# raulmur/ORB_SLAM2

Hardware: AMD Instinct MI355X
Metric: frames/s ORB extract+match, 1241x376 gray, 2000 kpts, 8 lvls (higher is better)
Workload: dtype u8

## Files before the change

orb_slam2_amd/csrc/orbhip_api.hip:

```cpp
#include <cstdarg>
#include <unistd.h>
#include <sys/syscall.h>
#include "orbhip_ctx.h"

static thread_local std::string g_err;
orbhip_status orbhip_set_error(orbhip_status st, const char* fmt, ...)
{
    char buf[512]; va_list ap; va_start(ap, fmt); vsnprintf(buf, sizeof buf, fmt, ap); va_end(ap);
    g_err = buf; return st;
}

static const char* kKernelNames[K_COUNT] = {"k_pyramid_level", "k_fast_cells", "k_blur", "k_quadtree", "k_describe",
                                            "k_match_grid", "k_match_candidates", "k_match_select", "k_undistort_keys", "k_remap"};

static const signed char kPatternHost[256 * 4] = {
#include "brief_pattern_31.inc"
};

void prof_collect(orbhip_ctx* c)
{
    for (auto& s : c->pending) {
        (void)hipEventSynchronize(s.b);
        float ms = 0; (void)hipEventElapsedTime(&ms, s.a, s.b);
        c->tot_ms[s.k] += ms; c->launches[s.k] += s.counts;
// ... 557 lines not shown

orbhip_status run_pipeline(orbhip_ctx* c, int nimg, const uint8_t* d_img0, long long frame_stride, int row_stride,
                           int match_prev, int window, float nnratio, int check_ori)
{
    orbhip_status st = begin_batch(c, d_img0, frame_stride, row_stride); if (st != ORBHIP_OK) return st;
    const int cur = c->cur, prev = (cur + 2) % 3;
    const int ngroups = std::min((int)c->xstreams.size() + 1, nimg);
    ExtractParams P = make_params(c, d_img0, frame_stride, row_stride);
    if (ngroups > 1) { HIPCHK(hipEventRecord(c->ev_fork, c->stream)); }
    for (int gi = 0; gi < ngroups; gi++) {
        const int f0 = (int)((long long)nimg * gi / ngroups), f1 = (int)((long long)nimg * (gi + 1) / ngroups), nf = f1 - f0;
        hipStream_t s = gi == 0 ? c->stream : c->xstreams[gi - 1];
        if (gi > 0) HIPCHK(hipStreamWaitEvent(s, c->ev_fork, 0));
        if (nf <= 0) continue;
        st = pipeline_frames(c, P, f0, nf, s, ngroups == 1); if (st != ORBHIP_OK) return st;
        if (gi > 0) { HIPCHK(hipEventRecord(c->xevents[gi - 1], s)); HIPCHK(hipStreamWaitEvent(c->stream, c->xevents[gi - 1], 0)); }
    }
    if (match_prev) {
        MatchParams M; memset(&M, 0, sizeof M);
        M.kp1 = c->distorted ? c->d_out_kpun[prev] : c->d_out_kp[prev]; M.desc1 = c->d_out_desc[prev]; M.n1 = c->d_out_n[prev]; M.n1_lvl0 = c->d_lvl_n[prev];
        M.kp2 = c->distorted ? c->d_out_kpun[cur] : c->d_out_kp[cur]; M.desc2 = c->d_out_desc[cur]; M.n2 = c->d_out_n[cur];
        M.lvl_stride = c->L; M.list1 = nullptr; M.prev_from_kp1 = 1;
        M.cap = c->out_cap; M.min_x = c->bounds.min_x; M.min_y = c->bounds.min_y; M.max_x = c->bounds.max_x; M.max_y = c->bounds.max_y;
        M.grid_start = c->d_grid_start; M.grid_items = c->d_grid_items; M.grid_xy = c->d_grid_xy; M.cand = c->d_cand; M.top = c->d_top; M.ncand = c->d_ncand; M.cand_stride = c->lvl0_cap; M.lvl0_cap = c->lvl0_cap;
        M.prev = c->d_prev; M.matches12 = c->d_m12; M.nmatches = c->d_nm; M.window = window; M.nnratio = nnratio; M.check_ori = check_ori; M.slot0 = 0;
        if (orbhip_match_select_big(c->out_cap, c->lvl0_cap)) {
            if (!c->d_match_ws) HIPCHK(dalloc(&c->d_match_ws, (size_t)c->B * orbhip_match_select_ints(c->out_cap, c->lvl0_cap)));
            M.big_ws = c->d_match_ws;
        }
        hipStream_t ms = c->serial ? c->stream : c->mstream;
        HIPCHK(hipEventRecord(c->ev_extract, c->stream));
        HIPCHK(hipStreamWaitEvent(ms, c->ev_extract, 0));
        { ProfScope ps(c, K_MGRID, ms); orbhip_launch_match_grid(M, nimg, ms); }
        { ProfScope ps(c, K_MCAND, ms); orbhip_launch_match_candidates(M, nimg, ms); }
        { ProfScope ps(c, K_MSELECT, ms); orbhip_launch_match_select(M, nimg, ms); }
        HIPCHK(hipEventRecord(c->ev_match[cur], ms));
        c->match_pending[cur] = true;
    }
    c->last_matched = match_prev != 0;
    c->last_nimg = nimg;
    HIPCHK(hipGetLastError());
    return ORBHIP_OK;
}

extern "C" orbhip_status orbhip_extract_device(orbhip_ctx* c, int nimg, const uint8_t* d_imgs, size_t frame_stride, int row_stride,
                                               int match_prev, int window, float nnratio, int check_ori)
{
    if (!c || !d_imgs) return fail(ORBHIP_ERR_INVALID, "null argument");
    if (nimg < 1 || nimg > c->B) return fail(ORBHIP_ERR_INVALID, "nimg %d outside 1..%d", nimg, c->B);
    if (row_stride < c->cfg.width) return fail(ORBHIP_ERR_INVALID, "row stride %d < width %d", row_stride, c->cfg.width);
// ... 133 lines not shown
```

orb_slam2_amd/csrc/orbhip_internal.h:

```cpp
#pragma once
#include <hip/hip_runtime.h>
#include <cstdint>
#include "../../include/orbhip.h"

#include <cstdlib>
inline hipError_t orbhip_dmalloc(void** p, size_t bytes)
{
    const hipError_t e = hipMalloc(p, bytes);
    if (e != hipSuccess) return e;
    static const int poison = [] { const char* v = getenv("ORBHIP_POISON"); return v && *v ? atoi(v) & 255 : -1; }();
    if (poison < 0) return hipSuccess;
    const hipError_t m = hipMemset(*p, poison, bytes);
    return m != hipSuccess ? m : hipDeviceSynchronize();
}

#define ORBHIP_MAX_LEVELS 16
#define ORBHIP_QT_DEPTH 13
#define ORBHIP_GRID_COLS 64
#define ORBHIP_GRID_ROWS 48
#define ORBHIP_GRID_CELLS (ORBHIP_GRID_COLS * ORBHIP_GRID_ROWS)
#define ORBHIP_HISTO_LENGTH 30
#define ORBHIP_TH_LOW 50
#define ORBHIP_EDGE 16

// ... 43 lines not shown
    const float* patternf;
    int iniTh, minTh, blur_round_mode, fp_contract;
    int qt_maxn;
    int qt_maxcells;
    int qt_scr;
    int fc_pstride, fc_prows, fc_sstride, fc_srows, fc_listcap;
    int fc_cell0, fc_ncells;
    int fc_pbytes, fc_np; const int4* fc_dma;
    const short2* pc_xr; const short2* pc_yr; int pc_ntx, pc_nty, pc_buf0, pc_buf1, pc_xcap, pc_ycap;
};

struct MatchParams {
    const orbhip_keypoint* kp1; const uint8_t* desc1; const int* n1;
    const int* n1_lvl0; int lvl_stride;
    const int* list1;
    int prev_from_kp1;
    const orbhip_keypoint* kp2; const uint8_t* desc2; const int* n2;
    int cap;
    float min_x, min_y, max_x, max_y;
    int* grid_start; int* grid_items; float2* grid_xy;
    unsigned* cand; int* ncand; int cand_stride;
    unsigned* top;
    int lvl0_cap;
    float* prev;
    int* matches12; int* nmatches;
    int window; float nnratio; int check_ori;
    int slot0;
    int grid_all_levels;
    int* big_ws;
};
size_t orbhip_match_select_ints(int cap, int lvl0_cap);
bool orbhip_match_select_big(int cap, int lvl0_cap);

struct StereoSide {
    const orbhip_keypoint* kp; const uint8_t* desc; const int* n;
    const uint8_t* img0; long long img0_frame_stride; int img0_pitch;
    const uint8_t* pyr; long long plane_frame_bytes;
};
struct StereoParams {
    const LevelGeom* geom; StereoSide L, R;
    int cap, im_h;
    int* row_start; int* row_items; int row_cap;
    float* u_right; float* depth; int* sad;
    float mbf, maxD;
};
hipError_t orbhip_copy_async(void* dst, const void* src, size_t bytes, hipMemcpyKind kind, hipStream_t s);
int orbhip_device_numa_node(int device);
bool orbhip_bind_thread_to_node(int node);
void orbhip_launch_stereo(const StereoParams& T, int nslots, int max_left, hipStream_t s, bool rows_ready = false);
void orbhip_launch_stereo_rows(const StereoParams& T, int nslots, hipStream_t s);

struct ProjParams {
    const orbhip_keypoint* kp; const uint8_t* desc; const float* u_right; int n;
    float min_x, min_y, max_x, max_y;
    const int* grid_start; const int* grid_items; const float2* grid_xy;
// ... 142 lines not shown
```

orb_slam2_amd/csrc/orbhip_kernels_match.hip:

```cpp
#include "orbhip_internal.h"
#include <cstdlib>
#include <cstring>
#include <type_traits>

#define WAVE 64
#define IMAX 0x7fffffff

#define NN_T 256
#define NN_QPT 4
#define NN_ROWS 256
#define NN_CHUNK 8192

struct NNPart { int best, second; long long idx; };

__global__ __launch_bounds__(NN_T) void k_hamming_nn(const unsigned long long* q, int nq, const unsigned long long* db, long long ndb,
                                                     long long base, NNPart* parts, int nchunks)
{
    __shared__ unsigned long long s_db[NN_ROWS * 4];
    const int tid = threadIdx.x, chunk = blockIdx.y;
    const int q0 = (blockIdx.x * NN_T + tid) * NN_QPT;
    unsigned long long qa[NN_QPT][4];
    unsigned kb[NN_QPT], ks[NN_QPT];
#pragma unroll
    for (int k = 0; k < NN_QPT; k++) {
// ... 444 lines not shown
    const float gwInv = (float)ORBHIP_GRID_COLS / (float)(M.max_x - M.min_x), ghInv = (float)ORBHIP_GRID_ROWS / (float)(M.max_y - M.min_y);
    size_t lds_max = (size_t)150 * 1024;
#ifdef ORBHIP_TEST_HOOKS
    if (const char* e = getenv("ORBHIP_TEST_MATCH_GRID_LDS_MAX")) lds_max = (size_t)atol(e);
#endif
    if (orbhip_match_grid_lds(M.cap) <= lds_max) hipLaunchKernelGGL(k_match_grid, dim3(nslots, 1, 1), dim3(256, 1, 1), orbhip_match_grid_lds(M.cap), s, M, gwInv, ghInv);
    else hipLaunchKernelGGL(k_match_grid_big, dim3(nslots, 1, 1), dim3(256, 1, 1), 0, s, M, gwInv, ghInv);
}

__device__ __forceinline__ int wave_min_dpp(int v)
{
    v = min(v, __builtin_amdgcn_update_dpp(IMAX, v, 0x111, 0xf, 0xf, false));
    v = min(v, __builtin_amdgcn_update_dpp(IMAX, v, 0x112, 0xf, 0xf, false));
    v = min(v, __builtin_amdgcn_update_dpp(IMAX, v, 0x114, 0xf, 0xe, false));
    v = min(v, __builtin_amdgcn_update_dpp(IMAX, v, 0x118, 0xf, 0xc, false));
    v = min(v, __builtin_amdgcn_update_dpp(IMAX, v, 0x142, 0xa, 0xf, false));
    v = min(v, __builtin_amdgcn_update_dpp(IMAX, v, 0x143, 0xc, 0xf, false));
    return __builtin_amdgcn_readlane(v, 63);
}

#define MS_K 4
#define MS_REC (MS_K + 1)
#define MS_NONE 0xFFFFFFFFu
#define MC_CHUNKS 8
__global__ __launch_bounds__(256) void k_match_candidates(MatchParams M, float gwInv, float ghInv)
{
    const int wave = __builtin_amdgcn_readfirstlane(threadIdx.x >> 6), lane = threadIdx.x & 63, slot = blockIdx.y + M.slot0;
    const int j1 = blockIdx.x * 4 + wave;
    const int n1l = M.n1_lvl0[slot * M.lvl_stride];
    if (j1 >= n1l || j1 >= M.lvl0_cap) return;
    const int i1 = M.list1 ? M.list1[(long long)slot * M.lvl0_cap + j1] : j1;
    const int nitems = M.grid_start[(long long)slot * (ORBHIP_GRID_CELLS + 1) + ORBHIP_GRID_CELLS];
    const int* gitems = M.grid_items + (long long)slot * M.cap;
    const float2* gxy = M.grid_xy + (long long)slot * M.cap;
    unsigned* cand = M.cand + ((long long)slot * M.lvl0_cap + j1) * M.cand_stride;
    const orbhip_keypoint* kp1 = M.kp1 + (long long)slot * M.cap;
    const float x = M.prev_from_kp1 ? kp1[i1].x : M.prev[((long long)slot * M.cap + i1) * 2];
    const float y = M.prev_from_kp1 ? kp1[i1].y : M.prev[((long long)slot * M.cap + i1) * 2 + 1];
    const float r = (float)M.window;
    const unsigned long long* d1 = (const unsigned long long*)(M.desc1 + ((long long)slot * M.cap + i1) * 32);
    const unsigned long long q0 = d1[0], q1 = d1[1], q2 = d1[2], q3 = d1[3];
    const unsigned long long below = (1ull << lane) - 1ull;
    int nc = 0;
    int tk[MS_K]; unsigned te[MS_K]; int nsel = 0;
#pragma unroll
    for (int k = 0; k < MS_K; k++) { tk[k] = IMAX; te[k] = MS_NONE; }
    const int* gstart = M.grid_start + (long long)slot * (ORBHIP_GRID_CELLS + 1);
    const float cl = __fmul_rn(__fsub_rn(__fsub_rn(x, M.min_x), r), gwInv), ch = __fmul_rn(__fadd_rn(__fsub_rn(x, M.min_x), r), gwInv);
    const int col_lo = cl >= 1.0f ? (int)fminf(floorf(cl) - 1.0f, (float)ORBHIP_GRID_COLS) : 0;
    const int col_hi = ch < (float)(ORBHIP_GRID_COLS - 2) ? (int)fmaxf(ceilf(ch) + 2.0f, 0.0f) : ORBHIP_GRID_COLS;
    const int t_lo = __builtin_amdgcn_readfirstlane(gstart[min(col_lo, col_hi) * ORBHIP_GRID_ROWS]), t_hi = __builtin_amdgcn_readfirstlane(gstart[col_hi * ORBHIP_GRID_ROWS]);
    (void)nitems;
    for (int tb = t_lo; tb < t_hi; tb += 64 * MC_CHUNKS) {
        float2 k[MC_CHUNKS]; int it[MC_CHUNKS];
#pragma unroll
        for (int c = 0; c < MC_CHUNKS; c++) {
            const int t = tb + 64 * c + lane;
            k[c].x = 0.0f; k[c].y = 0.0f; it[c] = 0;
            if (t < t_hi) { k[c] = gxy[t]; it[c] = gitems[t]; }
        }
#pragma unroll
        for (int c = 0; c < MC_CHUNKS; c++) {
            if (tb + 64 * c >= t_hi) break;
            const bool ok = tb + 64 * c + lane < t_hi && fabsf(__fsub_rn(k[c].x, x)) < r && fabsf(__fsub_rn(k[c].y, y)) < r;
            const unsigned long long m = __ballot(ok);
            if (m == 0) continue;
            const int pos = nc + __popcll(m & below);
            if (ok && pos < M.cand_stride) {
                const unsigned long long* d2 = (const unsigned long long*)(M.desc2 + ((long long)slot * M.cap + it[c]) * 32);
                const int dist = __popcll(q0 ^ d2[0]) + __popcll(q1 ^ d2[1]) + __popcll(q2 ^ d2[2]) + __popcll(q3 ^ d2[3]);
                unsigned rec = (unsigned)it[c] | ((unsigned)dist << 20);
                cand[pos] = rec;
                int key = (dist << 20) | pos;
                nsel++;
#pragma unroll
                for (int k = 0; k < MS_K; k++) if (key < tk[k]) { const int tkk = tk[k]; const unsigned tee = te[k]; tk[k] = key; te[k] = rec; key = tkk; rec = tee; }
            }
            nc += __popcll(m);
        }
    }
    nc = min(nc, M.cand_stride);
    if (lane == 0) M.ncand[(long long)slot * M.lvl0_cap + j1] = nc;
    unsigned out = MS_NONE; int popped = 0;
#pragma unroll
    for (int r = 0; r < MS_K; r++) {
        const int m = wave_min_dpp(tk[0]);
        if (m == IMAX) break;
        const int owner = __ffsll((long long)__ballot(tk[0] == m)) - 1;
        const unsigned rec = (unsigned)__builtin_amdgcn_readlane((int)te[0], owner);
        if (lane == r) out = rec;
        if (lane == owner) {
            popped++;
#pragma unroll
            for (int k = 0; k + 1 < MS_K; k++) { tk[k] = tk[k + 1]; te[k] = te[k + 1]; }
            tk[MS_K - 1] = IMAX; te[MS_K - 1] = MS_NONE;
        }
    }
    const bool more = __ballot(nsel > popped) != 0ull;
    unsigned* top = M.top + ((long long)slot * M.lvl0_cap + j1) * MS_REC;
    if (lane < MS_K) top[lane] = out;
    if (lane == MS_K) top[MS_K] = more ? 1u : 0u;
}

void orbhip_launch_match_candidates(const MatchParams& M, int nslots, hipStream_t s)
{
    const float gwInv = (float)ORBHIP_GRID_COLS / (float)(M.max_x - M.min_x), ghInv = (float)ORBHIP_GRID_ROWS / (float)(M.max_y - M.min_y);
    hipLaunchKernelGGL(k_match_candidates, dim3((M.lvl0_cap + 3) / 4, nslots, 1), dim3(256, 1, 1), 0, s, M, gwInv, ghInv);
}


#define MS_T 256

__device__ __forceinline__ int orbhip_match_select_ints_d(int cap, int lvl0_cap) { return 4 * cap + 4 * lvl0_cap + ORBHIP_HISTO_LENGTH + 8; }
template <bool BIG> __device__ __forceinline__ void match_select_body(const MatchParams& M)
{
    typedef typename std::conditional<BIG, volatile int, int>::type TI;
    typedef typename std::conditional<BIG, volatile float, float>::type TF;
    const int slot = blockIdx.x + M.slot0, tid = threadIdx.x, lane = tid & 63, wave = tid >> 6;
    const int n1 = M.n1[slot], n2 = M.n2[slot];
    const int n1l = min(M.n1_lvl0[slot * M.lvl_stride], M.lvl0_cap);
    const int* list1 = M.list1 ? M.list1 + (long long)slot * M.lvl0_cap : nullptr;
    HIP_DYNAMIC_SHARED(int, lds)
    TI* s_md = BIG ? M.big_ws + (long long)(blockIdx.x + M.slot0) * (long long)orbhip_match_select_ints_d(M.cap, M.lvl0_cap) : lds;
    TI* s_m21 = s_md + M.cap;
    TI* s_m12 = s_m21 + M.cap;
    TI* s_bin = s_m12 + M.lvl0_cap;
    TI* s_nc = s_bin + M.lvl0_cap;
    TI* s_hist = s_nc + M.lvl0_cap;
    TI* s_stamp = s_hist + ORBHIP_HISTO_LENGTH + 8;
    TF* s_ang1 = reinterpret_cast<TF*>(s_stamp + M.cap);
    TF* s_ang2 = s_ang1 + M.lvl0_cap;
    auto amin = [](TI* p, int v) { atomicMin(const_cast<int*>(p), v); };
    auto aadd = [](TI* p, int v) { atomicAdd(const_cast<int*>(p), v); };
    const orbhip_keypoint* kp1 = M.kp1 + (long long)slot * M.cap;
    const orbhip_keypoint* kp2 = M.kp2 + (long long)slot * M.cap;
    int* m12 = M.matches12 + (long long)slot * M.cap;
    float* prev = M.prev + (long long)slot * M.cap * 2;
    const unsigned* cand0 = M.cand + (long long)slot * M.lvl0_cap * M.cand_stride;
    for (int i = tid; i < n2; i += MS_T) { s_md[i] = IMAX; s_m21[i] = -1; s_stamp[i] = IMAX; s_ang2[i] = kp2[i].angle; }
    for (int i = tid; i < n1l; i += MS_T) { s_m12[i] = -1; s_bin[i] = -1; s_nc[i] = M.ncand[(long long)slot * M.lvl0_cap + i]; s_ang1[i] = kp1[list1 ? list1[i] : i].angle; }
    for (int i = tid; i < ORBHIP_HISTO_LENGTH + 8; i += MS_T) s_hist[i] = 0;
    for (int i = tid; i < n1; i += MS_T) { m12[i] = -1; if (M.prev_from_kp1) { prev[2 * i] = kp1[i].x; prev[2 * i + 1] = kp1[i].y; } }
    __syncthreads();
    if (wave == 0) {
        const float factor = 1.0f / ORBHIP_HISTO_LENGTH;
        const unsigned* top0 = M.top + (long long)slot * M.lvl0_cap * MS_REC;
        auto rot_bin = [&](int j1, int i2) -> int {
            float rot = __fsub_rn(s_ang1[j1], s_ang2[i2]);
            if (rot < 0.0f) rot = __fadd_rn(rot, 360.0f);
            int bin = (int)roundf(__fmul_rn(rot, factor));
            if (bin == ORBHIP_HISTO_LENGTH) bin = 0;
            return min(max(bin, 0), ORBHIP_HISTO_LENGTH - 1);
        };
        for (int jb = 0; jb < n1l; jb += 64) {
            const int j1 = jb + lane;
            const bool inb = j1 < n1l;
            int ei[MS_K], ed[MS_K]; int nk = 0;
#pragma unroll
            for (int k = 0; k < MS_K; k++) {
                const unsigned t = (inb && s_nc[j1] != 0) ? top0[(long long)j1 * MS_REC + k] : MS_NONE;
                ei[k] = (int)(t & 0xFFFFFu); ed[k] = (int)((t >> 20) & 0x1FFu);
                if (t != MS_NONE) nk = k + 1;
            }
            const bool more = nk > 0 && top0[(long long)j1 * MS_REC + MS_K] != 0u;
            int stamped = -1;
            unsigned long long todo = __ballot(nk > 0);
            while (todo) {
                const bool mine = (todo >> lane) & 1ull;
                const int lowest = __ffsll((long long)todo) - 1;
                int a = -1, b = -1;
#pragma unroll
                for (int k = 0; k < MS_K; k++)
                    if (mine && k < nk && b < 0 && !(s_md[ei[k]] <= ed[k])) { if (a < 0) a = k; else b = k; }
                const int ia = a >= 0 ? ei[a] : 0, da = a >= 0 ? ed[a] : IMAX, db = b >= 0 ? ed[b] : IMAX;
                const bool exhausted = mine && more && b < 0;
                const bool accept = mine && !exhausted && a >= 0 && da <= ORBHIP_TH_LOW && (float)da < __fmul_rn((float)db, M.nnratio);
                const int want = accept ? ia : -1;
                if (stamped >= 0 && stamped != want && s_stamp[stamped] == j1) s_stamp[stamped] = IMAX;
                __builtin_amdgcn_wave_barrier();
                if (want >= 0) amin(&s_stamp[want], j1);
                stamped = want;
                __builtin_amdgcn_wave_barrier();
                bool unsure = false;
                const int last = b >= 0 ? b : nk - 1;
#pragma unroll
                for (int k = 0; k < MS_K; k++)
                    if (mine && lane != lowest && k <= last && !(s_md[ei[k]] <= ed[k]) && s_stamp[ei[k]] < j1) unsure = true;
                const unsigned long long bad = __ballot(unsure || exhausted);
                const int first_bad = bad ? __ffsll((long long)bad) - 1 : 64;
                const unsigned long long commit = first_bad == 64 ? todo : (todo & ((1ull << first_bad) - 1ull));
                const bool win = ((commit >> lane) & 1ull) && accept;
                if (win) {
                    const int old = s_m21[ia];
                    if (old >= 0) s_m12[old] = -1;
                    s_m12[j1] = ia; s_m21[ia] = j1; s_md[ia] = da;
                    if (s_stamp[ia] == j1) s_stamp[ia] = IMAX;
                    stamped = -1;
                    if (M.check_ori) { const int bin = rot_bin(j1, ia); s_bin[j1] = bin; aadd(&s_hist[bin], 1); }
                }
                __builtin_amdgcn_wave_barrier();
                todo &= ~commit;
                if (first_bad == 64) break;
                if (first_bad != lowest || !((__ballot(exhausted) >> first_bad) & 1ull)) continue;
                todo &= ~(1ull << first_bad);
                if (lane == first_bad && stamped >= 0 && s_stamp[stamped] == j1) s_stamp[stamped] = IMAX;
                const int js = jb + first_bad, nc = s_nc[js];
                const unsigned* cand = cand0 + (long long)js * M.cand_stride;
                int best = IMAX, second = IMAX, bidx = -1;
                for (int cb = 0; cb < nc; cb += 64) {
                    const int t = cb + lane;
                    const unsigned e = t < nc ? cand[t] : 0u;
                    const int i2 = (int)(e & 0xFFFFFu), dist = (int)(e >> 20);
                    const bool valid = t < nc && !(s_md[i2] <= dist);
                    const int key = valid ? ((dist << 6) | lane) : IMAX;
                    const int k1 = wave_min_dpp(key);
                    if (k1 == IMAX) continue;
                    const int first = k1 & 63, wmin = k1 >> 6, ci = __builtin_amdgcn_readlane(i2, first);
                    const int k2 = wave_min_dpp(lane == first ? IMAX : key);
                    const int wsec = k2 == IMAX ? IMAX : (k2 >> 6);
                    if (wmin < best) { second = min(best, wsec); best = wmin; bidx = ci; } else second = min(second, wmin);
                }
                if (best <= ORBHIP_TH_LOW && (float)best < __fmul_rn((float)second, M.nnratio)) {
                    if (lane == 0) {
                        const int old = s_m21[bidx];
                        if (old >= 0) s_m12[old] = -1;
                        s_m12[js] = bidx; s_m21[bidx] = js; s_md[bidx] = best;
                        if (M.check_ori) { const int bin = rot_bin(js, bidx); s_bin[js] = bin; s_hist[bin] = s_hist[bin] + 1; }
                    }
                }
                __builtin_amdgcn_wave_barrier();
            }
        }
    }
    if (wave != 0) return;
    __builtin_amdgcn_wave_barrier();
    if (M.check_ori) {
        if (lane == 0) {
            int max1 = 0, max2 = 0, max3 = 0, ind1 = -1, ind2 = -1, ind3 = -1;
            for (int i = 0; i < ORBHIP_HISTO_LENGTH; i++) {
                const int s = s_hist[i];
                if (s > max1) { max3 = max2; max2 = max1; max1 = s; ind3 = ind2; ind2 = ind1; ind1 = i; }
                else if (s > max2) { max3 = max2; max2 = s; ind3 = ind2; ind2 = i; }
                else if (s > max3) { max3 = s; ind3 = i; }
            }
            if ((float)max2 < __fmul_rn(0.1f, (float)max1)) { ind2 = -1; ind3 = -1; }
            else if ((float)max3 < __fmul_rn(0.1f, (float)max1)) { ind3 = -1; }
            s_hist[ORBHIP_HISTO_LENGTH] = ind1; s_hist[ORBHIP_HISTO_LENGTH + 1] = ind2; s_hist[ORBHIP_HISTO_LENGTH + 2] = ind3;
        }
        __builtin_amdgcn_wave_barrier();
        const int ind1 = s_hist[ORBHIP_HISTO_LENGTH], ind2 = s_hist[ORBHIP_HISTO_LENGTH + 1], ind3 = s_hist[ORBHIP_HISTO_LENGTH + 2];
        for (int j = lane; j < n1l; j += 64) { const int b = s_bin[j]; if (b >= 0 && b != ind1 && b != ind2 && b != ind3) s_m12[j] = -1; }
        __builtin_amdgcn_wave_barrier();
    }
    int cnt = 0;
    for (int j = lane; j < n1l; j += 64) {
        const int m = s_m12[j];
        if (m >= 0) { const int i1 = list1 ? list1[j] : j; cnt++; m12[i1] = m; prev[2 * i1] = kp2[m].x; prev[2 * i1 + 1] = kp2[m].y; }
    }
#pragma unroll
    for (int off = 32; off >= 1; off >>= 1) cnt += __shfl_xor(cnt, off);
    if (lane == 0) M.nmatches[slot] = cnt;
}

__global__ __launch_bounds__(MS_T) void k_match_select(MatchParams M) { match_select_body<false>(M); }
__global__ __launch_bounds__(MS_T) void k_match_select_big(MatchParams M) { match_select_body<true>(M); }

#define MS_LDS_BUDGET (158 * 1024)
size_t orbhip_match_select_ints(int cap, int lvl0_cap) { return (size_t)4 * cap + (size_t)4 * lvl0_cap + ORBHIP_HISTO_LENGTH + 8; }
bool orbhip_match_select_big(int cap, int lvl0_cap)
{
    const char* env = getenv("ORBHIP_SELECT_BIG");
    const bool force = env && env[0] == '1';
    return force || sizeof(int) * orbhip_match_select_ints(cap, lvl0_cap) > MS_LDS_BUDGET;
}
void orbhip_launch_match_select(const MatchParams& M, int nslots, hipStream_t s)
{
    if (M.big_ws) hipLaunchKernelGGL(k_match_select_big, dim3(nslots, 1, 1), dim3(MS_T, 1, 1), 0, s, M);
    else hipLaunchKernelGGL(k_match_select, dim3(nslots, 1, 1), dim3(MS_T, 1, 1), sizeof(int) * orbhip_match_select_ints(M.cap, M.lvl0_cap), s, M);
}
```

orb_slam2_amd/csrc/orbhip_search.hip:

```cpp
#include "orbhip_ctx.h"

static thread_local struct HeldSlots { int device = -1; size_t floor = 0; std::vector<BestParams> B; std::vector<int> live_of_slot; } g_held;

void launch_feature_grid(const orbhip_keypoint* kp, const int* d_n, int cap, const orbhip_bounds& b, int* grid_start, int* grid_items, float2* grid_xy,
                         int nslots, int slot0, hipStream_t s)
{
    MatchParams M; memset(&M, 0, sizeof M);
    M.kp2 = kp; M.n2 = d_n; M.cap = cap; M.min_x = b.min_x; M.min_y = b.min_y; M.max_x = b.max_x; M.max_y = b.max_y;
    M.grid_start = grid_start; M.grid_items = grid_items; M.grid_xy = grid_xy; M.grid_all_levels = 1; M.slot0 = slot0;
    orbhip_launch_match_grid(M, nslots, s);
}

static bool projection_ok(const orbhip_projection* P)
{
    const int kind = P ? P->kind & ~ORBHIP_FP_CONTRACT : -1;
    return P && kind >= ORBHIP_PROJ_LAST_FRAME && kind <= ORBHIP_PROJ_SIM3 && P->gemm_mode >= 0 && P->gemm_mode <= 2 && P->nlevels >= 1 && P->nlevels <= ORBHIP_MAX_PROJ_LEVELS;
}
static bool fp_contract_of(const orbhip_projection* P) { return P && (P->kind & ORBHIP_FP_CONTRACT); }
static orbhip_projection bare_projection(const orbhip_projection& P) { orbhip_projection Q = P; Q.kind &= ~ORBHIP_FP_CONTRACT; return Q; }
template <typename Query> static void gated_out(Query* q, int np) { if (q) for (int i = 0; i < np; i++) { memset(&q[i], 0, sizeof q[i]); q[i].radius = -1.0f; } }
static void no_match(int32_t* best_idx, int32_t* best_dist, int nq) { for (int i = 0; i < nq; i++) { best_idx[i] = -1; best_dist[i] = 256; } }
template <typename T> static void arena_in(Arena& A, const T** p, const T* src, size_t count) { T* d = nullptr; A.io(&d, count, src, count); *p = d; }

struct SearchFrame {
// ... 474 lines not shown
    OrbApiTimer api_timer;
    if (n1 < 0 || n2 < 0 || !nmatches || (n1 > 0 && (!kps1 || !desc1 || !prev_matched || !matches12)) || (n2 > 0 && (!kps2 || !desc2)) || !bounds || !(bounds->max_x > bounds->min_x) || !(bounds->max_y > bounds->min_y))
        return fail(ORBHIP_ERR_INVALID, "bad argument");
    *nmatches = 0;
    for (int i = 0; i < n1; i++) matches12[i] = -1;
    if (n1 == 0) return ORBHIP_OK;
    if (!device_present()) return fail(ORBHIP_ERR_HIP, "no HIP device available: no CPU fallback");
    HIPCHK(hipSetDevice(device));
    hipStream_t ts = orbhip_thread_stream(device);
    std::vector<int> list1; for (int i = 0; i < n1; i++) if (kps1[i].octave <= 0) list1.push_back(i);
    int n2l0 = 0; for (int i = 0; i < n2; i++) n2l0 += kps2[i].octave == 0;
    const int cap = std::max(std::max(n1, n2), 1), l0cap = std::max((int)list1.size(), 1), cstride = std::max(n2l0, 1);
    orbhip_keypoint *dk1 = nullptr, *dk2 = nullptr; uint8_t *dd1 = nullptr, *dd2 = nullptr; int *dn = nullptr, *dlist = nullptr, *dgs = nullptr, *dgi = nullptr, *dnc = nullptr, *dm12 = nullptr, *dbig = nullptr; float2* dgxy = nullptr;
    unsigned* dcand = nullptr; unsigned* dtop = nullptr; float* dprev = nullptr;
    const int hn[4] = {n1, n2, (int)list1.size(), 0}; int hres[4] = {0, 0, 0, 0};
    const hipError_t e = arena_call(device, ts, [&](Arena& A) {
        A.io(&dk1, cap, kps1, n1); A.io(&dk2, cap, kps2, n2); A.io(&dd1, (size_t)cap * 32, desc1, (size_t)n1 * 32); A.io(&dd2, (size_t)cap * 32, desc2, (size_t)n2 * 32);
        A.io(&dlist, l0cap, (const int*)list1.data(), list1.size());
        A.io(&dn, 8, hn, 4, hres, 4);
        A.io(&dprev, (size_t)cap * 2, (const float*)prev_matched, (size_t)n1 * 2, prev_matched, (size_t)n1 * 2);
        A.io(&dm12, cap, (const int*)nullptr, 0, matches12, n1);
        A.take(&dgs, ORBHIP_GRID_CELLS + 1); A.take(&dgi, cap); A.take(&dgxy, cap); A.take(&dnc, l0cap);
        A.take(&dcand, (size_t)l0cap * cstride); A.take(&dtop, (size_t)l0cap * 5);
        if (orbhip_match_select_big(cap, l0cap)) A.take(&dbig, orbhip_match_select_ints(cap, l0cap));
    }, [&] {
        MatchParams M; memset(&M, 0, sizeof M);
        M.kp1 = dk1; M.desc1 = dd1; M.n1 = dn; M.n1_lvl0 = dn + 2; M.kp2 = dk2; M.desc2 = dd2; M.n2 = dn + 1; M.lvl_stride = 0; M.list1 = dlist; M.prev_from_kp1 = 0;
        M.cap = cap; M.min_x = bounds->min_x; M.min_y = bounds->min_y; M.max_x = bounds->max_x; M.max_y = bounds->max_y; M.grid_start = dgs; M.grid_items = dgi; M.grid_xy = dgxy; M.cand = dcand; M.top = dtop; M.ncand = dnc; M.cand_stride = cstride; M.lvl0_cap = l0cap;
        M.prev = dprev; M.matches12 = dm12; M.nmatches = dn + 3; M.window = window; M.nnratio = nnratio; M.check_ori = check_ori; M.big_ws = dbig;
        orbhip_launch_match_grid(M, 1, ts); orbhip_launch_match_candidates(M, 1, ts); orbhip_launch_match_select(M, 1, ts);
    });
    if (e != hipSuccess) return fail(ORBHIP_ERR_HIP, "search_for_initialization: %s", hipGetErrorString(e));
    *nmatches = hres[3];
    return ORBHIP_OK;
}

static bool whole_image(int im_w, int im_h, orbhip_bounds* b) { if (im_w < 1 || im_h < 1) return false; b->min_x = 0.0f; b->min_y = 0.0f; b->max_x = (float)im_w; b->max_y = (float)im_h; return true; }
extern "C" orbhip_status orbhip_search_by_projection(int device, const orbhip_keypoint* kps, const uint8_t* desc, const float* u_right, const uint8_t* blocked, int n,
                                                     int im_w, int im_h, const orbhip_proj_query* queries, const uint8_t* query_desc, int nq,
                                                     int mode, float nnratio, int th_high, int check_ori, int32_t* feature_query, int* nmatches)
{
    orbhip_bounds b; if (!whole_image(im_w, im_h, &b)) return fail(ORBHIP_ERR_INVALID, "bad argument");
    return orbhip_search_by_projection_bounds(device, kps, desc, u_right, blocked, n, &b, queries, query_desc, nq, mode, nnratio, th_high, check_ori, feature_query, nmatches);
}
extern "C" orbhip_status orbhip_search_best_in_window(int device, const orbhip_keypoint* kps, const uint8_t* desc, const float* u_right, int n, int im_w, int im_h,
                                                      const float* inv_level_sigma2, int nlevels, const orbhip_best_query* queries, const uint8_t* query_desc, int nq,
                                                      int chi2_gate, int32_t* best_idx, int32_t* best_dist)
{
    orbhip_bounds b; if (!whole_image(im_w, im_h, &b)) return fail(ORBHIP_ERR_INVALID, "bad argument");
    return orbhip_search_best_in_window_bounds(device, kps, desc, u_right, n, &b, inv_level_sigma2, nlevels, queries, query_desc, nq, chi2_gate, best_idx, best_dist);
}
// ... 55 lines not shown
```

Measured before the change: 206,800.

## Pack match candidates per 16-lane row and compact select-stage state tables

The candidate kernel now handles four level-0 keypoints per wave, one per 16-lane row. It uses a row-wide DPP min reduction instead of a whole-wave one and launches a quarter as many blocks. Candidate records now store the grid-table index instead of the keypoint index. This lets the select kernel keep one packed dist/match word per table entry plus one packed accept/bin word per query, cutting its LDS footprint and init work. The select kernel shrinks to a single 64-thread wave. The new tab_cap clamp and the packed bit fields add risk of truncation or index overflow when counts are large.

New measurement: 209,100 (median of 6 runs). 1.01x the previous value.

```diff
diff --git a/orb_slam2_amd/csrc/orbhip_api.hip b/orb_slam2_amd/csrc/orbhip_api.hip
--- a/orb_slam2_amd/csrc/orbhip_api.hip
+++ b/orb_slam2_amd/csrc/orbhip_api.hip
@@ -603,10 +603,10 @@
         M.kp2 = c->distorted ? c->d_out_kpun[cur] : c->d_out_kp[cur]; M.desc2 = c->d_out_desc[cur]; M.n2 = c->d_out_n[cur];
         M.lvl_stride = c->L; M.list1 = nullptr; M.prev_from_kp1 = 1;
         M.cap = c->out_cap; M.min_x = c->bounds.min_x; M.min_y = c->bounds.min_y; M.max_x = c->bounds.max_x; M.max_y = c->bounds.max_y;
-        M.grid_start = c->d_grid_start; M.grid_items = c->d_grid_items; M.grid_xy = c->d_grid_xy; M.cand = c->d_cand; M.top = c->d_top; M.ncand = c->d_ncand; M.cand_stride = c->lvl0_cap; M.lvl0_cap = c->lvl0_cap;
+        M.grid_start = c->d_grid_start; M.grid_items = c->d_grid_items; M.grid_xy = c->d_grid_xy; M.cand = c->d_cand; M.top = c->d_top; M.ncand = c->d_ncand; M.cand_stride = c->lvl0_cap; M.lvl0_cap = c->lvl0_cap; M.tab_cap = c->lvl0_cap;
         M.prev = c->d_prev; M.matches12 = c->d_m12; M.nmatches = c->d_nm; M.window = window; M.nnratio = nnratio; M.check_ori = check_ori; M.slot0 = 0;
-        if (orbhip_match_select_big(c->out_cap, c->lvl0_cap)) {
-            if (!c->d_match_ws) HIPCHK(dalloc(&c->d_match_ws, (size_t)c->B * orbhip_match_select_ints(c->out_cap, c->lvl0_cap)));
+        if (orbhip_match_select_big(c->lvl0_cap, c->lvl0_cap)) {
+            if (!c->d_match_ws) HIPCHK(dalloc(&c->d_match_ws, (size_t)c->B * orbhip_match_select_ints(c->lvl0_cap, c->lvl0_cap)));
             M.big_ws = c->d_match_ws;
         }
         hipStream_t ms = c->serial ? c->stream : c->mstream;
diff --git a/orb_slam2_amd/csrc/orbhip_internal.h b/orb_slam2_amd/csrc/orbhip_internal.h
--- a/orb_slam2_amd/csrc/orbhip_internal.h
+++ b/orb_slam2_amd/csrc/orbhip_internal.h
@@ -89,6 +89,7 @@
     unsigned* cand; int* ncand; int cand_stride;
     unsigned* top;
     int lvl0_cap;
+    int tab_cap;
     float* prev;
     int* matches12; int* nmatches;
     int window; float nnratio; int check_ori;
@@ -96,8 +97,8 @@
     int grid_all_levels;
     int* big_ws;
 };
-size_t orbhip_match_select_ints(int cap, int lvl0_cap);
-bool orbhip_match_select_big(int cap, int lvl0_cap);
+size_t orbhip_match_select_ints(int tab_cap, int lvl0_cap);
+bool orbhip_match_select_big(int tab_cap, int lvl0_cap);
 
 struct StereoSide {
     const orbhip_keypoint* kp; const uint8_t* desc; const int* n;
diff --git a/orb_slam2_amd/csrc/orbhip_kernels_match.hip b/orb_slam2_amd/csrc/orbhip_kernels_match.hip
--- a/orb_slam2_amd/csrc/orbhip_kernels_match.hip
+++ b/orb_slam2_amd/csrc/orbhip_kernels_match.hip
@@ -490,15 +490,25 @@
 #define MS_K 4
 #define MS_REC (MS_K + 1)
 #define MS_NONE 0xFFFFFFFFu
-#define MC_CHUNKS 8
+#define MC_CHUNKS 4
+#define MC_KPW 4
+__device__ __forceinline__ int row_min_dpp(int v)
+{
+    v = min(v, __builtin_amdgcn_update_dpp(IMAX, v, 0xB1, 0xf, 0xf, false));
+    v = min(v, __builtin_amdgcn_update_dpp(IMAX, v, 0x4E, 0xf, 0xf, false));
+    v = min(v, __builtin_amdgcn_update_dpp(IMAX, v, 0x141, 0xf, 0xf, false));
+    v = min(v, __builtin_amdgcn_update_dpp(IMAX, v, 0x128, 0xf, 0xf, false));
+    return v;
+}
 __global__ __launch_bounds__(256) void k_match_candidates(MatchParams M, float gwInv, float ghInv)
 {
     const int wave = __builtin_amdgcn_readfirstlane(threadIdx.x >> 6), lane = threadIdx.x & 63, slot = blockIdx.y + M.slot0;
-    const int j1 = blockIdx.x * 4 + wave;
-    const int n1l = M.n1_lvl0[slot * M.lvl_stride];
-    if (j1 >= n1l || j1 >= M.lvl0_cap) return;
+    const int row = lane >> 4, rl = lane & 15;
+    const int n1l = min(M.n1_lvl0[slot * M.lvl_stride], M.lvl0_cap);
+    if ((blockIdx.x * 4 + wave) * MC_KPW >= n1l) return;
+    const bool live = (blockIdx.x * 4 + wave) * MC_KPW + row < n1l;
+    const int j1 = live ? (blockIdx.x * 4 + wave) * MC_KPW + row : n1l - 1;
     const int i1 = M.list1 ? M.list1[(long long)slot * M.lvl0_cap + j1] : j1;
-    const int nitems = M.grid_start[(long long)slot * (ORBHIP_GRID_CELLS + 1) + ORBHIP_GRID_CELLS];
     const int* gitems = M.grid_items + (long long)slot * M.cap;
     const float2* gxy = M.grid_xy + (long long)slot * M.cap;
     unsigned* cand = M.cand + ((long long)slot * M.lvl0_cap + j1) * M.cand_stride;
@@ -508,7 +518,7 @@
     const float r = (float)M.window;
     const unsigned long long* d1 = (const unsigned long long*)(M.desc1 + ((long long)slot * M.cap + i1) * 32);
     const unsigned long long q0 = d1[0], q1 = d1[1], q2 = d1[2], q3 = d1[3];
-    const unsigned long long below = (1ull << lane) - 1ull;
+    const unsigned below = (1u << rl) - 1u;
     int nc = 0;
     int tk[MS_K]; unsigned te[MS_K]; int nsel = 0;
 #pragma unroll
@@ -517,192 +527,190 @@
     const float cl = __fmul_rn(__fsub_rn(__fsub_rn(x, M.min_x), r), gwInv), ch = __fmul_rn(__fadd_rn(__fsub_rn(x, M.min_x), r), gwInv);
     const int col_lo = cl >= 1.0f ? (int)fminf(floorf(cl) - 1.0f, (float)ORBHIP_GRID_COLS) : 0;
     const int col_hi = ch < (float)(ORBHIP_GRID_COLS - 2) ? (int)fmaxf(ceilf(ch) + 2.0f, 0.0f) : ORBHIP_GRID_COLS;
-    const int t_lo = __builtin_amdgcn_readfirstlane(gstart[min(col_lo, col_hi) * ORBHIP_GRID_ROWS]), t_hi = __builtin_amdgcn_readfirstlane(gstart[col_hi * ORBHIP_GRID_ROWS]);
-    (void)nitems;
-    for (int tb = t_lo; tb < t_hi; tb += 64 * MC_CHUNKS) {
+    const int t_lo = min(gstart[min(col_lo, col_hi) * ORBHIP_GRID_ROWS], M.tab_cap), t_hi = live ? min(gstart[col_hi * ORBHIP_GRID_ROWS], M.tab_cap) : 0;
+    for (int tb = t_lo + rl; __ballot(tb - rl < t_hi) != 0ull; tb += 16 * MC_CHUNKS) {
         float2 k[MC_CHUNKS]; int it[MC_CHUNKS];
 #pragma unroll
         for (int c = 0; c < MC_CHUNKS; c++) {
-            const int t = tb + 64 * c + lane;
+            const int t = tb + 16 * c;
             k[c].x = 0.0f; k[c].y = 0.0f; it[c] = 0;
             if (t < t_hi) { k[c] = gxy[t]; it[c] = gitems[t]; }
         }
 #pragma unroll
         for (int c = 0; c < MC_CHUNKS; c++) {
-            if (tb + 64 * c >= t_hi) break;
-            const bool ok = tb + 64 * c + lane < t_hi && fabsf(__fsub_rn(k[c].x, x)) < r && fabsf(__fsub_rn(k[c].y, y)) < r;
+            const int t = tb + 16 * c;
+            const bool ok = t < t_hi && fabsf(__fsub_rn(k[c].x, x)) < r && fabsf(__fsub_rn(k[c].y, y)) < r;
             const unsigned long long m = __ballot(ok);
             if (m == 0) continue;
-            const int pos = nc + __popcll(m & below);
+            const unsigned mr = (unsigned)(m >> (16 * row)) & 0xFFFFu;
+            const int pos = nc + __popc(mr & below);
             if (ok && pos < M.cand_stride) {
                 const unsigned long long* d2 = (const unsigned long long*)(M.desc2 + ((long long)slot * M.cap + it[c]) * 32);
                 const int dist = __popcll(q0 ^ d2[0]) + __popcll(q1 ^ d2[1]) + __popcll(q2 ^ d2[2]) + __popcll(q3 ^ d2[3]);
-                unsigned rec = (unsigned)it[c] | ((unsigned)dist << 20);
+                unsigned rec = (unsigned)t | ((unsigned)dist << 20);
                 cand[pos] = rec;
                 int key = (dist << 20) | pos;
                 nsel++;
 #pragma unroll
                 for (int k = 0; k < MS_K; k++) if (key < tk[k]) { const int tkk = tk[k]; const unsigned tee = te[k]; tk[k] = key; te[k] = rec; key = tkk; rec = tee; }
             }
-            nc += __popcll(m);
+            nc += __popc(mr);
         }
     }
     nc = min(nc, M.cand_stride);
-    if (lane == 0) M.ncand[(long long)slot * M.lvl0_cap + j1] = nc;
-    unsigned out = MS_NONE; int popped = 0;
+    if (live && rl == 0) M.ncand[(long long)slot * M.lvl0_cap + j1] = nc;
+    unsigned* top = M.top + ((long long)slot * M.lvl0_cap + j1) * MS_REC;
+    int popped = 0, nrec = 0;
 #pragma unroll
     for (int r = 0; r < MS_K; r++) {
-        const int m = wave_min_dpp(tk[0]);
-        if (m == IMAX) break;
-        const int owner = __ffsll((long long)__ballot(tk[0] == m)) - 1;
-        const unsigned rec = (unsigned)__builtin_amdgcn_readlane((int)te[0], owner);
-        if (lane == r) out = rec;
-        if (lane == owner) {
+        const int m = row_min_dpp(tk[0]);
+        if (m != IMAX) nrec = r + 1;
+        if (m != IMAX && tk[0] == m) {
+            if (live) top[r] = te[0];
             popped++;
 #pragma unroll
             for (int k = 0; k + 1 < MS_K; k++) { tk[k] = tk[k + 1]; te[k] = te[k + 1]; }
             tk[MS_K - 1] = IMAX; te[MS_K - 1] = MS_NONE;
         }
     }
-    const bool more = __ballot(nsel > popped) != 0ull;
-    unsigned* top = M.top + ((long long)slot * M.lvl0_cap + j1) * MS_REC;
-    if (lane < MS_K) top[lane] = out;
-    if (lane == MS_K) top[MS_K] = more ? 1u : 0u;
+    const bool more = ((unsigned)(__ballot(nsel > popped) >> (16 * row)) & 0xFFFFu) != 0u;
+    if (live && rl >= nrec && rl < MS_K) top[rl] = MS_NONE;
+    if (live && rl == MS_K) top[MS_K] = more ? 1u : 0u;
 }
 
 void orbhip_launch_match_candidates(const MatchParams& M, int nslots, hipStream_t s)
 {
     const float gwInv = (float)ORBHIP_GRID_COLS / (float)(M.max_x - M.min_x), ghInv = (float)ORBHIP_GRID_ROWS / (float)(M.max_y - M.min_y);
-    hipLaunchKernelGGL(k_match_candidates, dim3((M.lvl0_cap + 3) / 4, nslots, 1), dim3(256, 1, 1), 0, s, M, gwInv, ghInv);
-}
-
-
-#define MS_T 256
-
-__device__ __forceinline__ int orbhip_match_select_ints_d(int cap, int lvl0_cap) { return 4 * cap + 4 * lvl0_cap + ORBHIP_HISTO_LENGTH + 8; }
+    hipLaunchKernelGGL(k_match_candidates, dim3((M.lvl0_cap + 4 * MC_KPW - 1) / (4 * MC_KPW), nslots, 1), dim3(256, 1, 1), 0, s, M, gwInv, ghInv);
+}
+
+
+#define MS_T 64
+
+#define MS_MD_NONE 0x3FF
+#define MS_J_MASK 0x1FFFFF
+__device__ __forceinline__ int orbhip_match_select_ints_d(int tab_cap, int lvl0_cap) { return 2 * tab_cap + lvl0_cap + ORBHIP_HISTO_LENGTH + 8; }
 template <bool BIG> __device__ __forceinline__ void match_select_body(const MatchParams& M)
 {
     typedef typename std::conditional<BIG, volatile int, int>::type TI;
-    typedef typename std::conditional<BIG, volatile float, float>::type TF;
-    const int slot = blockIdx.x + M.slot0, tid = threadIdx.x, lane = tid & 63, wave = tid >> 6;
-    const int n1 = M.n1[slot], n2 = M.n2[slot];
+    const int slot = blockIdx.x + M.slot0, lane = threadIdx.x;
+    const int n1 = M.n1[slot];
     const int n1l = min(M.n1_lvl0[slot * M.lvl_stride], M.lvl0_cap);
     const int* list1 = M.list1 ? M.list1 + (long long)slot * M.lvl0_cap : nullptr;
+    const int nt = min(M.grid_start[(long long)slot * (ORBHIP_GRID_CELLS + 1) + ORBHIP_GRID_CELLS], M.tab_cap);
     HIP_DYNAMIC_SHARED(int, lds)
-    TI* s_md = BIG ? M.big_ws + (long long)(blockIdx.x + M.slot0) * (long long)orbhip_match_select_ints_d(M.cap, M.lvl0_cap) : lds;
-    TI* s_m21 = s_md + M.cap;
-    TI* s_m12 = s_m21 + M.cap;
-    TI* s_bin = s_m12 + M.lvl0_cap;
-    TI* s_nc = s_bin + M.lvl0_cap;
-    TI* s_hist = s_nc + M.lvl0_cap;
-    TI* s_stamp = s_hist + ORBHIP_HISTO_LENGTH + 8;
-    TF* s_ang1 = reinterpret_cast<TF*>(s_stamp + M.cap);
-    TF* s_ang2 = s_ang1 + M.lvl0_cap;
+    TI* s_mdm = BIG ? M.big_ws + (long long)slot * (long long)orbhip_match_select_ints_d(M.tab_cap, M.lvl0_cap) : lds;
+    TI* s_stamp = s_mdm + M.tab_cap;
+    TI* s_acc = s_stamp + M.tab_cap;
+    TI* s_hist = s_acc + M.lvl0_cap;
     auto amin = [](TI* p, int v) { atomicMin(const_cast<int*>(p), v); };
     auto aadd = [](TI* p, int v) { atomicAdd(const_cast<int*>(p), v); };
     const orbhip_keypoint* kp1 = M.kp1 + (long long)slot * M.cap;
     const orbhip_keypoint* kp2 = M.kp2 + (long long)slot * M.cap;
+    const int* gitems = M.grid_items + (long long)slot * M.cap;
+    const float2* gxy = M.grid_xy + (long long)slot * M.cap;
+    const int* ncand = M.ncand + (long long)slot * M.lvl0_cap;
     int* m12 = M.matches12 + (long long)slot * M.cap;
     float* prev = M.prev + (long long)slot * M.cap * 2;
     const unsigned* cand0 = M.cand + (long long)slot * M.lvl0_cap * M.cand_stride;
-    for (int i = tid; i < n2; i += MS_T) { s_md[i] = IMAX; s_m21[i] = -1; s_stamp[i] = IMAX; s_ang2[i] = kp2[i].angle; }
-    for (int i = tid; i < n1l; i += MS_T) { s_m12[i] = -1; s_bin[i] = -1; s_nc[i] = M.ncand[(long long)slot * M.lvl0_cap + i]; s_ang1[i] = kp1[list1 ? list1[i] : i].angle; }
-    for (int i = tid; i < ORBHIP_HISTO_LENGTH + 8; i += MS_T) s_hist[i] = 0;
-    for (int i = tid; i < n1; i += MS_T) { m12[i] = -1; if (M.prev_from_kp1) { prev[2 * i] = kp1[i].x; prev[2 * i + 1] = kp1[i].y; } }
-    __syncthreads();
-    if (wave == 0) {
+    const unsigned* top0 = M.top + (long long)slot * M.lvl0_cap * MS_REC;
+    for (int t = lane; t < nt; t += MS_T) { s_mdm[t] = MS_MD_NONE << 21; s_stamp[t] = IMAX; }
+    for (int i = lane; i < n1l; i += MS_T) s_acc[i] = 0;
+    for (int i = lane; i < ORBHIP_HISTO_LENGTH + 8; i += MS_T) s_hist[i] = 0;
+    for (int i = lane; i < n1; i += MS_T) { m12[i] = -1; if (M.prev_from_kp1) { prev[2 * i] = kp1[i].x; prev[2 * i + 1] = kp1[i].y; } }
+    __syncthreads();
+    auto matched_dist = [&](int t) -> int { return s_mdm[t] >> 21; };
+    auto accept_match = [&](int j1, int t, int dist) {
+        const int old = (s_mdm[t] & MS_J_MASK) - 1;
+        if (old >= 0) s_acc[old] = s_acc[old] & ~32;
+        s_acc[j1] = ((t + 1) << 6) | 32; s_mdm[t] = (dist << 21) | (j1 + 1);
+    };
+    for (int jb = 0; jb < n1l; jb += 64) {
+        const int j1 = jb + lane;
+        const bool inb = j1 < n1l;
+        int ei[MS_K], ed[MS_K]; int nk = 0;
+        const bool any = inb && ncand[j1] != 0;
+#pragma unroll
+        for (int k = 0; k < MS_K; k++) {
+            const unsigned t = any ? top0[(long long)j1 * MS_REC + k] : MS_NONE;
+            ei[k] = (int)(t & 0xFFFFFu); ed[k] = (int)((t >> 20) & 0x1FFu);
+            if (t != MS_NONE) nk = k + 1;
+        }
+        const bool more = nk > 0 && top0[(long long)j1 * MS_REC + MS_K] != 0u;
+        int stamped = -1;
+        unsigned long long todo = __ballot(nk > 0);
+        while (todo) {
+            const bool mine = (todo >> lane) & 1ull;
+            const int lowest = __ffsll((long long)todo) - 1;
+            int a = -1, b = -1;
+#pragma unroll
+            for (int k = 0; k < MS_K; k++)
+                if (mine && k < nk && b < 0 && !(matched_dist(ei[k]) <= ed[k])) { if (a < 0) a = k; else b = k; }
+            const int ia = a >= 0 ? ei[a] : 0, da = a >= 0 ? ed[a] : IMAX, db = b >= 0 ? ed[b] : IMAX;
+            const bool exhausted = mine && more && b < 0;
+            const bool accept = mine && !exhausted && a >= 0 && da <= ORBHIP_TH_LOW && (float)da < __fmul_rn((float)db, M.nnratio);
+            const int want = accept ? ia : -1;
+            if (stamped >= 0 && stamped != want && s_stamp[stamped] == j1) s_stamp[stamped] = IMAX;
+            __builtin_amdgcn_wave_barrier();
+            if (want >= 0) amin(&s_stamp[want], j1);
+            stamped = want;
+            __builtin_amdgcn_wave_barrier();
+            bool unsure = false;
+            const int last = b >= 0 ? b : nk - 1;
+#pragma unroll
+            for (int k = 0; k < MS_K; k++)
+                if (mine && lane != lowest && k <= last && !(matched_dist(ei[k]) <= ed[k]) && s_stamp[ei[k]] < j1) unsure = true;
+            const unsigned long long bad = __ballot(unsure || exhausted);
+            const int first_bad = bad ? __ffsll((long long)bad) - 1 : 64;
+            const unsigned long long commit = first_bad == 64 ? todo : (todo & ((1ull << first_bad) - 1ull));
+            const bool win = ((commit >> lane) & 1ull) && accept;
+            if (win) {
+                accept_match(j1, ia, da);
+                if (s_stamp[ia] == j1) s_stamp[ia] = IMAX;
+                stamped = -1;
+            }
+            __builtin_amdgcn_wave_barrier();
+            todo &= ~commit;
+            if (first_bad == 64) break;
+            if (first_bad != lowest || !((__ballot(exhausted) >> first_bad) & 1ull)) continue;
+            todo &= ~(1ull << first_bad);
+            if (lane == first_bad && stamped >= 0 && s_stamp[stamped] == j1) s_stamp[stamped] = IMAX;
+            const int js = jb + first_bad, nc = ncand[js];
+            const unsigned* cand = cand0 + (long long)js * M.cand_stride;
+            int best = IMAX, second = IMAX, bidx = -1;
+            for (int cb = 0; cb < nc; cb += 64) {
+                const int c = cb + lane;
+                const unsigned e = c < nc ? cand[c] : 0u;
+                const int t = (int)(e & 0xFFFFFu), dist = (int)(e >> 20);
+                const bool valid = c < nc && !(matched_dist(t) <= dist);
+                const int key = valid ? ((dist << 6) | lane) : IMAX;
+                const int k1 = wave_min_dpp(key);
+                if (k1 == IMAX) continue;
+                const int first = k1 & 63, wmin = k1 >> 6, ci = __builtin_amdgcn_readlane(t, first);
+                const int k2 = wave_min_dpp(lane == first ? IMAX : key);
+                const int wsec = k2 == IMAX ? IMAX : (k2 >> 6);
+                if (wmin < best) { second = min(best, wsec); best = wmin; bidx = ci; } else second = min(second, wmin);
+            }
+            if (best <= ORBHIP_TH_LOW && (float)best < __fmul_rn((float)second, M.nnratio)) {
+                if (lane == 0) accept_match(js, bidx, best);
+            }
+            __builtin_amdgcn_wave_barrier();
+        }
+    }
+    __builtin_amdgcn_wave_barrier();
+    if (M.check_ori) {
         const float factor = 1.0f / ORBHIP_HISTO_LENGTH;
-        const unsigned* top0 = M.top + (long long)slot * M.lvl0_cap * MS_REC;
-        auto rot_bin = [&](int j1, int i2) -> int {
-            float rot = __fsub_rn(s_ang1[j1], s_ang2[i2]);
+        for (int j = lane; j < n1l; j += 64) {
+            const int w = s_acc[j];
+            if (w == 0) continue;
+            float rot = __fsub_rn(kp1[list1 ? list1[j] : j].angle, kp2[gitems[(w >> 6) - 1]].angle);
             if (rot < 0.0f) rot = __fadd_rn(rot, 360.0f);
             int bin = (int)roundf(__fmul_rn(rot, factor));
             if (bin == ORBHIP_HISTO_LENGTH) bin = 0;
-            return min(max(bin, 0), ORBHIP_HISTO_LENGTH - 1);
-        };
-        for (int jb = 0; jb < n1l; jb += 64) {
-            const int j1 = jb + lane;
-            const bool inb = j1 < n1l;
-            int ei[MS_K], ed[MS_K]; int nk = 0;
-#pragma unroll
-            for (int k = 0; k < MS_K; k++) {
-                const unsigned t = (inb && s_nc[j1] != 0) ? top0[(long long)j1 * MS_REC + k] : MS_NONE;
-                ei[k] = (int)(t & 0xFFFFFu); ed[k] = (int)((t >> 20) & 0x1FFu);
-                if (t != MS_NONE) nk = k + 1;
-            }
-            const bool more = nk > 0 && top0[(long long)j1 * MS_REC + MS_K] != 0u;
-            int stamped = -1;
-            unsigned long long todo = __ballot(nk > 0);
-            while (todo) {
-                const bool mine = (todo >> lane) & 1ull;
-                const int lowest = __ffsll((long long)todo) - 1;
-                int a = -1, b = -1;
-#pragma unroll
-                for (int k = 0; k < MS_K; k++)
-                    if (mine && k < nk && b < 0 && !(s_md[ei[k]] <= ed[k])) { if (a < 0) a = k; else b = k; }
-                const int ia = a >= 0 ? ei[a] : 0, da = a >= 0 ? ed[a] : IMAX, db = b >= 0 ? ed[b] : IMAX;
-                const bool exhausted = mine && more && b < 0;
-                const bool accept = mine && !exhausted && a >= 0 && da <= ORBHIP_TH_LOW && (float)da < __fmul_rn((float)db, M.nnratio);
-                const int want = accept ? ia : -1;
-                if (stamped >= 0 && stamped != want && s_stamp[stamped] == j1) s_stamp[stamped] = IMAX;
-                __builtin_amdgcn_wave_barrier();
-                if (want >= 0) amin(&s_stamp[want], j1);
-                stamped = want;
-                __builtin_amdgcn_wave_barrier();
-                bool unsure = false;
-                const int last = b >= 0 ? b : nk - 1;
-#pragma unroll
-                for (int k = 0; k < MS_K; k++)
-                    if (mine && lane != lowest && k <= last && !(s_md[ei[k]] <= ed[k]) && s_stamp[ei[k]] < j1) unsure = true;
-                const unsigned long long bad = __ballot(unsure || exhausted);
-                const int first_bad = bad ? __ffsll((long long)bad) - 1 : 64;
-                const unsigned long long commit = first_bad == 64 ? todo : (todo & ((1ull << first_bad) - 1ull));
-                const bool win = ((commit >> lane) & 1ull) && accept;
-                if (win) {
-                    const int old = s_m21[ia];
-                    if (old >= 0) s_m12[old] = -1;
-                    s_m12[j1] = ia; s_m21[ia] = j1; s_md[ia] = da;
-                    if (s_stamp[ia] == j1) s_stamp[ia] = IMAX;
-                    stamped = -1;
-                    if (M.check_ori) { const int bin = rot_bin(j1, ia); s_bin[j1] = bin; aadd(&s_hist[bin], 1); }
-                }
-                __builtin_amdgcn_wave_barrier();
-                todo &= ~commit;
-                if (first_bad == 64) break;
-                if (first_bad != lowest || !((__ballot(exhausted) >> first_bad) & 1ull)) continue;
-                todo &= ~(1ull << first_bad);
-                if (lane == first_bad && stamped >= 0 && s_stamp[stamped] == j1) s_stamp[stamped] = IMAX;
-                const int js = jb + first_bad, nc = s_nc[js];
-                const unsigned* cand = cand0 + (long long)js * M.cand_stride;
-                int best = IMAX, second = IMAX, bidx = -1;
-                for (int cb = 0; cb < nc; cb += 64) {
-                    const int t = cb + lane;
-                    const unsigned e = t < nc ? cand[t] : 0u;
-                    const int i2 = (int)(e & 0xFFFFFu), dist = (int)(e >> 20);
-                    const bool valid = t < nc && !(s_md[i2] <= dist);
-                    const int key = valid ? ((dist << 6) | lane) : IMAX;
-                    const int k1 = wave_min_dpp(key);
-                    if (k1 == IMAX) continue;
-                    const int first = k1 & 63, wmin = k1 >> 6, ci = __builtin_amdgcn_readlane(i2, first);
-                    const int k2 = wave_min_dpp(lane == first ? IMAX : key);
-                    const int wsec = k2 == IMAX ? IMAX : (k2 >> 6);
-                    if (wmin < best) { second = min(best, wsec); best = wmin; bidx = ci; } else second = min(second, wmin);
-                }
-                if (best <= ORBHIP_TH_LOW && (float)best < __fmul_rn((float)second, M.nnratio)) {
-                    if (lane == 0) {
-                        const int old = s_m21[bidx];
-                        if (old >= 0) s_m12[old] = -1;
-                        s_m12[js] = bidx; s_m21[bidx] = js; s_md[bidx] = best;
-                        if (M.check_ori) { const int bin = rot_bin(js, bidx); s_bin[js] = bin; s_hist[bin] = s_hist[bin] + 1; }
-                    }
-                }
-                __builtin_amdgcn_wave_barrier();
-            }
-        }
-    }
-    if (wave != 0) return;
-    __builtin_amdgcn_wave_barrier();
-    if (M.check_ori) {
+            bin = min(max(bin, 0), ORBHIP_HISTO_LENGTH - 1);
+            s_acc[j] = w | bin; aadd(&s_hist[bin], 1);
+        }
+        __builtin_amdgcn_wave_barrier();
         if (lane == 0) {
             int max1 = 0, max2 = 0, max3 = 0, ind1 = -1, ind2 = -1, ind3 = -1;
             for (int i = 0; i < ORBHIP_HISTO_LENGTH; i++) {
@@ -716,14 +724,15 @@
             s_hist[ORBHIP_HISTO_LENGTH] = ind1; s_hist[ORBHIP_HISTO_LENGTH + 1] = ind2; s_hist[ORBHIP_HISTO_LENGTH + 2] = ind3;
         }
         __builtin_amdgcn_wave_barrier();
-        const int ind1 = s_hist[ORBHIP_HISTO_LENGTH], ind2 = s_hist[ORBHIP_HISTO_LENGTH + 1], ind3 = s_hist[ORBHIP_HISTO_LENGTH + 2];
-        for (int j = lane; j < n1l; j += 64) { const int b = s_bin[j]; if (b >= 0 && b != ind1 && b != ind2 && b != ind3) s_m12[j] = -1; }
-        __builtin_amdgcn_wave_barrier();
-    }
+    }
+    const int ind1 = s_hist[ORBHIP_HISTO_LENGTH], ind2 = s_hist[ORBHIP_HISTO_LENGTH + 1], ind3 = s_hist[ORBHIP_HISTO_LENGTH + 2];
     int cnt = 0;
     for (int j = lane; j < n1l; j += 64) {
-        const int m = s_m12[j];
-        if (m >= 0) { const int i1 = list1 ? list1[j] : j; cnt++; m12[i1] = m; prev[2 * i1] = kp2[m].x; prev[2 * i1 + 1] = kp2[m].y; }
+        const int w = s_acc[j], b = w & 31;
+        if (!(w & 32) || (M.check_ori && b != ind1 && b != ind2 && b != ind3)) continue;
+        const int t = (w >> 6) - 1, i1 = list1 ? list1[j] : j;
+        const float2 xy = gxy[t];
+        cnt++; m12[i1] = gitems[t]; prev[2 * i1] = xy.x; prev[2 * i1 + 1] = xy.y;
     }
 #pragma unroll
     for (int off = 32; off >= 1; off >>= 1) cnt += __shfl_xor(cnt, off);
@@ -734,15 +743,15 @@
 __global__ __launch_bounds__(MS_T) void k_match_select_big(MatchParams M) { match_select_body<true>(M); }
 
 #define MS_LDS_BUDGET (158 * 1024)
-size_t orbhip_match_select_ints(int cap, int lvl0_cap) { return (size_t)4 * cap + (size_t)4 * lvl0_cap + ORBHIP_HISTO_LENGTH + 8; }
-bool orbhip_match_select_big(int cap, int lvl0_cap)
+size_t orbhip_match_select_ints(int tab_cap, int lvl0_cap) { return (size_t)2 * tab_cap + (size_t)lvl0_cap + ORBHIP_HISTO_LENGTH + 8; }
+bool orbhip_match_select_big(int tab_cap, int lvl0_cap)
 {
     const char* env = getenv("ORBHIP_SELECT_BIG");
     const bool force = env && env[0] == '1';
-    return force || sizeof(int) * orbhip_match_select_ints(cap, lvl0_cap) > MS_LDS_BUDGET;
+    return force || sizeof(int) * orbhip_match_select_ints(tab_cap, lvl0_cap) > MS_LDS_BUDGET;
 }
 void orbhip_launch_match_select(const MatchParams& M, int nslots, hipStream_t s)
 {
     if (M.big_ws) hipLaunchKernelGGL(k_match_select_big, dim3(nslots, 1, 1), dim3(MS_T, 1, 1), 0, s, M);
-    else hipLaunchKernelGGL(k_match_select, dim3(nslots, 1, 1), dim3(MS_T, 1, 1), sizeof(int) * orbhip_match_select_ints(M.cap, M.lvl0_cap), s, M);
-}
+    else hipLaunchKernelGGL(k_match_select, dim3(nslots, 1, 1), dim3(MS_T, 1, 1), sizeof(int) * orbhip_match_select_ints(M.tab_cap, M.lvl0_cap), s, M);
+}
diff --git a/orb_slam2_amd/csrc/orbhip_search.hip b/orb_slam2_amd/csrc/orbhip_search.hip
--- a/orb_slam2_amd/csrc/orbhip_search.hip
+++ b/orb_slam2_amd/csrc/orbhip_search.hip
@@ -520,11 +520,11 @@
         A.io(&dm12, cap, (const int*)nullptr, 0, matches12, n1);
         A.take(&dgs, ORBHIP_GRID_CELLS + 1); A.take(&dgi, cap); A.take(&dgxy, cap); A.take(&dnc, l0cap);
         A.take(&dcand, (size_t)l0cap * cstride); A.take(&dtop, (size_t)l0cap * 5);
-        if (orbhip_match_select_big(cap, l0cap)) A.take(&dbig, orbhip_match_select_ints(cap, l0cap));
+        if (orbhip_match_select_big(cstride, l0cap)) A.take(&dbig, orbhip_match_select_ints(cstride, l0cap));
     }, [&] {
         MatchParams M; memset(&M, 0, sizeof M);
         M.kp1 = dk1; M.desc1 = dd1; M.n1 = dn; M.n1_lvl0 = dn + 2; M.kp2 = dk2; M.desc2 = dd2; M.n2 = dn + 1; M.lvl_stride = 0; M.list1 = dlist; M.prev_from_kp1 = 0;
-        M.cap = cap; M.min_x = bounds->min_x; M.min_y = bounds->min_y; M.max_x = bounds->max_x; M.max_y = bounds->max_y; M.grid_start = dgs; M.grid_items = dgi; M.grid_xy = dgxy; M.cand = dcand; M.top = dtop; M.ncand = dnc; M.cand_stride = cstride; M.lvl0_cap = l0cap;
+        M.cap = cap; M.min_x = bounds->min_x; M.min_y = bounds->min_y; M.max_x = bounds->max_x; M.max_y = bounds->max_y; M.grid_start = dgs; M.grid_items = dgi; M.grid_xy = dgxy; M.cand = dcand; M.top = dtop; M.ncand = dnc; M.cand_stride = cstride; M.lvl0_cap = l0cap; M.tab_cap = cstride;
         M.prev = dprev; M.matches12 = dm12; M.nmatches = dn + 3; M.window = window; M.nnratio = nnratio; M.check_ori = check_ori; M.big_ws = dbig;
         orbhip_launch_match_grid(M, 1, ts); orbhip_launch_match_candidates(M, 1, ts); orbhip_launch_match_select(M, 1, ts);
     });
```
